# GBATZOLIS/ID-diff

Hardware: AMD Instinct MI355X
Metric: score-vector evals/sec (rows of S per second incl. the per-point spectrum), 32x32 ncsnpp (higher is better)
Workload: dtype f32 (3x3 convs: Winograd, fp32 transforms, contraction on pairs of fp16 values -- 22 significand bits, 3 products, fp32 accumulate (F(4,3) along the rows x 3 filter rows); 1x1/attention/dense contractions: fp32 operands split exactly into 3 bf16, 6 partial products, fp32 accumulate; the q/k/v projec

## Files before the change

id-diff_amd/_lib.py:

```python
import ctypes
import os
import subprocess

import torch

_HERE = os.path.dirname(os.path.abspath(__file__))
_VARIANT = os.environ.get("IDIFF_LIB_VARIANT", "")
_LIB_PATH = os.path.join(_HERE, "csrc", f"libidiff_hip.{_VARIANT}.so" if _VARIANT else "libidiff_hip.so")
_lib = None

ACT = {None: 0, "none": 0, "linear": 0, "silu": 1, "swish": 1, "elu": 2, "relu": 3, "lrelu": 4}

c_i, c_i64, c_f, c_p = ctypes.c_int, ctypes.c_int64, ctypes.c_float, ctypes.c_void_p


class Epilogue(ctypes.Structure):
    _fields_ = [("bias", c_p), ("rowbias", c_p), ("ld_rowbias", c_i64), ("rows_per_group", c_i), ("act", c_i),
                ("residual", c_p), ("ld_residual", c_i64), ("out_scale", c_f), ("rowscale", c_p), ("colstats", c_p)]


_SIGNATURES = {
    "idiff_abi_version": (c_i, []),
    "idiff_last_error": (ctypes.c_char_p, []),
    "idiff_source_stamp": (ctypes.c_char_p, []),
# ... 29 lines not shown
    "idiff_winograd43_pack_f32": (c_i, [c_p, c_p, c_i, c_i, c_p]),
    "idiff_conv2d_winograd43_f32": (c_i, [c_p, c_p, c_p, c_i, c_i, c_i, c_i, c_i, ctypes.POINTER(Epilogue), c_p]),
    "idiff_conv2d_winograd43h_ok": (c_i, [c_i] * 5),
    "idiff_winograd43h_weight_floats": (c_i64, [c_i, c_i]),
    "idiff_winograd43h_pack_f32": (c_i, [c_p, c_p, c_i, c_i, c_p]),
    "idiff_conv2d_winograd43h_f32": (c_i, [c_p, c_p, c_p, c_i, c_i, c_i, c_i, c_i, ctypes.POINTER(Epilogue), c_p]),
    "idiff_conv2d_wino1d_ok": (c_i, [c_i] * 5),
    "idiff_conv2d_wino1d_colstats_split": (c_i, [c_i] * 5),
    "idiff_wino1d_weight_floats": (c_i64, [c_i, c_i]),
    "idiff_wino1d_pack_f32": (c_i, [c_p, c_p, c_i, c_i, c_p]),
    "idiff_conv2d_wino1d_f32": (c_i, [c_p, c_p, c_p, c_i, c_i, c_i, c_i, c_i, ctypes.POINTER(Epilogue), c_p]),
    "idiff_conv2d_wino1d_gn_ok": (c_i, [c_i] * 6),
    "idiff_conv2d_wino1d_gn_f32": (c_i, [c_p, c_p, c_p, c_i, c_i, c_i, c_i, c_i, ctypes.POINTER(Epilogue), c_i, c_p, c_p, c_f, c_i, c_p]),
    "idiff_conv2d_winograd_split_ok": (c_i, [c_i] * 5),
    "idiff_winograd_split_weight_floats": (c_i64, [c_i, c_i]),
    "idiff_winograd_pack_split_f32": (c_i, [c_p, c_p, c_i, c_i, c_p]),
    "idiff_conv2d_winograd_split_f32": (c_i, [c_p, c_p, c_p] + [c_i] * 5 + [ctypes.POINTER(Epilogue), c_p]),
    "idiff_groupnorm_finalize_f32": (c_i, [c_p, c_i, c_i, c_p, c_i, c_i, c_i, c_i, c_i, c_f, c_p, c_p]),
    "idiff_groupnorm_nsplit": (c_i, [c_i, c_i, c_i]),
    "idiff_groupnorm_stats_f32": (c_i, [c_p, c_i, c_p, c_i, c_i, c_i, c_i, c_f, c_p, c_p, c_p]),
    "idiff_groupnorm_apply_f32": (c_i, [c_p, c_i, c_p, c_i, c_i, c_i, c_i, c_p, c_p, c_p, c_p, c_i64, c_i, c_p, c_p]),
    "idiff_groupnorm_apply_colstats_f32": (c_i, [c_p, c_i, c_p, c_i, c_i, c_i, c_i, c_p, c_i, c_p, c_i, c_f, c_p, c_p, c_p, c_i64,
                                                 c_i, c_p, c_p]),
    "idiff_softmax_rows_f32": (c_i, [c_p, c_p, c_i64, c_i, c_f, c_p]),
    "idiff_attention256_ok": (c_i, [c_i, c_i, c_i]),
    "idiff_attention256_f32": (c_i, [c_p, c_i64, c_p, c_p, c_p, c_p, c_p, c_i, c_i, c_i, c_f, c_p]),
    "idiff_attention_heads_ok": (c_i, [c_i, c_i, c_i, c_i]),
    "idiff_attention_heads_f32": (c_i, [c_p, c_i64, c_p, c_p, c_p, c_p, c_p, c_i, c_i, c_i, c_i, c_f, c_p]),
    "idiff_affine_act_f32": (c_i, [c_p, c_p, c_i64, c_f, c_f, c_i, c_p, c_i64, c_p]),
    "idiff_add_scale_f32": (c_i, [c_p, c_p, c_p, c_i64, c_f, c_p]),
    "idiff_fourier_embed_f32": (c_i, [c_p, c_p, c_p, c_i, c_i, c_p]),
    "idiff_positional_embed_f32": (c_i, [c_p, c_p, c_i, c_i, c_f, c_i, c_p]),
    "idiff_concat_cols_f32": (c_i, [c_p, c_i, c_p, c_i, c_p, c_i64, c_p]),
    "idiff_nchw_to_nhwc_f32": (c_i, [c_p, c_p, c_i, c_i, c_i, c_i, c_f, c_f, c_p]),
    "idiff_nhwc_to_nchw_f32": (c_i, [c_p, c_p, c_i, c_i, c_i, c_i, c_p, c_p]),
    "idiff_resample2x_nhwc_f32": (c_i, [c_p, c_p, c_i, c_i, c_i, c_i, c_i, c_p]),
    "idiff_perturb_f32": (c_i, [c_p, c_p, c_p, c_p, c_p, c_i64, c_i64, c_p]),
    "idiff_perturb_randn_f32": (c_i, [c_p, c_p, c_p, c_p, c_i64, c_i64, c_i64, ctypes.c_uint64, c_p, c_p]),
    "idiff_spectrum_workspace_bytes": (c_i64, [c_i, c_i, c_i]),
    "idiff_spectrum_f32": (c_i, [c_p, c_i, c_i, c_i, c_p, c_i64, c_p, c_p, c_p]),
    "idiff_colmean_f64": (c_i, [c_p, c_i, c_i, c_i, c_p, c_p, c_p]),
    "idiff_centered_gram_f64": (c_i, [c_p, c_p, c_i, c_i, c_i, c_p, c_p]),
    "idiff_centered_gram_rows_f64": (c_i, [c_p, c_p, c_i, c_i, c_i, c_i, c_p, c_p]),
    "idiff_symmetrize_upper_f64": (c_i, [c_p, c_i, c_p]),
    "idiff_symtridiag_scratch_doubles": (c_i64, [c_i]),
    "idiff_symband_ld": (c_i, []),
# ... 417 lines not shown
def groupnorm_nsplit(B, HW, C):
    return lib().idiff_groupnorm_nsplit(B, HW, C)


def groupnorm_stats(x, C, x2, C2, B, HW, G, eps, workspace, stats):
    _check(lib().idiff_groupnorm_stats_f32(x.data_ptr(), C, _ptr(x2), C2, B, HW, G, eps, workspace.data_ptr(),
                                           stats.data_ptr(), _stream()), "idiff_groupnorm_stats_f32")


def groupnorm_apply(x, C, x2, C2, B, HW, G, stats, gamma, beta, act, y, mod=None):
    _check(lib().idiff_groupnorm_apply_f32(x.data_ptr(), C, _ptr(x2), C2, B, HW, G, stats.data_ptr(), gamma.data_ptr(),
                                           beta.data_ptr(), _ptr(mod), mod.stride(0) if mod is not None else 0,
                                           ACT[act], y.data_ptr(), _stream()),
           "idiff_groupnorm_apply_f32")


def groupnorm_apply_colstats(x, C, x2, C2, B, HW, G, ws1, ns1, ws2, ns2, eps, gamma, beta, act, y, mod=None):
    _check(lib().idiff_groupnorm_apply_colstats_f32(x.data_ptr(), C, _ptr(x2), C2, B, HW, G, ws1.data_ptr(), ns1, _ptr(ws2), ns2,
                                                    eps, gamma.data_ptr(), beta.data_ptr(), _ptr(mod),
                                                    mod.stride(0) if mod is not None else 0, ACT[act], y.data_ptr(), _stream()),
           "idiff_groupnorm_apply_colstats_f32")


def softmax_rows(x, y, rows, cols, scale):
    _check(lib().idiff_softmax_rows_f32(x.data_ptr(), y.data_ptr(), rows, cols, scale, _stream()),
           "idiff_softmax_rows_f32")


def attention256_ok(B, tokens, C):
    return bool(lib().idiff_attention256_ok(B, tokens, C))


def pairs_scale_from_rows(w, bias=None, extra=1.0):
    ms = (w.double() ** 2).sum(dim=1).mean() * float(extra) ** 2
    if bias is not None:
        ms = ms + (bias.double() ** 2).mean()
    e = torch.round(-0.5 * torch.log2(ms.clamp_min(1e-300))).clamp(-24, 24)
    s = torch.exp2(e)
    return torch.stack([s, 1.0 / s]).to(torch.float32).contiguous()


def attention256(qk, vt, out, B, C, s_qk, s_v, scale, bias_v=None):
    _dev(qk, "qk"); _dev(vt, "vt"); _dev(out, "out"); _dev(s_qk, "s_qk"); _dev(s_v, "s_v")
    if qk.shape != (B * 256, 2 * C) or vt.shape != (B, C, 256) or out.numel() != B * 256 * C:
        raise RuntimeError(f"attention256: shapes qk {tuple(qk.shape)}, vt {tuple(vt.shape)}, out {tuple(out.shape)} for B = {B}, C = {C}")
    _check(lib().idiff_attention256_f32(qk.data_ptr(), qk.stride(0), vt.data_ptr(), _ptr(bias_v), s_qk.data_ptr(), s_v.data_ptr(),
# ... 264 lines not shown
```

id-diff_amd/csrc/common.h:

```cpp
#pragma once
#include <hip/hip_runtime.h>
#include <stdint.h>
#include <stdio.h>
#include <stdarg.h>

#include "../../include/idiff_hip.h"

#define IDIFF_API extern "C" __attribute__((visibility("default")))

namespace idiff {

void set_error(const char *fmt, ...);

inline int fail(const char *fmt, ...) {
  char buf[512];
  va_list ap;
  va_start(ap, fmt);
  vsnprintf(buf, sizeof(buf), fmt, ap);
  va_end(ap);
  set_error("%s", buf);
  return IDIFF_EINVAL;
}

inline int launch_status(const char *what) {
  hipError_t e = hipGetLastError();
  if (e != hipSuccess) {
    set_error("%s: %s", what, hipGetErrorString(e));
    return (int)e;
  }
  return 0;
}

enum Option { OPT_NO_WINOGRAD, OPT_NO_COLSTATS, OPT_NO_PIPE, OPT_SCALAR_EPILOGUE, OPT_DBUF_ONLY, OPT_TRIDIAG_ONESTAGE,
              OPT_UFD_ROWS, OPT_CHASE_WAVEFRONT, OPT_WINO_NGROUP, OPT_GRAM_SMALL_TILES, OPT_CHASE_SPIN_LIMIT, OPT_FAKE_CU_COUNT,
              OPT_SBR_SYNC, OPT_SBR_FULL, OPT_NO_SPLIT, OPT_WINO_SPLIT, OPT_SBR_LOOKAHEAD, OPT_NO_WINO43, OPT_NO_WINO43H, OPT_NO_PAIRS, OPT_PAIRS_MIN_TILES, OPT_NO_FUSED_ATTN, OPT_NO_WINO1D, OPT_NO_FUSED_GN, OPT_COUNT };
bool option(Option o);
int option_value(Option o);

struct AttrGuard { unsigned long long done_mask = 0; };
int set_dynamic_lds_once(AttrGuard &g, const void *const *fns, int n_fns, int bytes, const char *what);

bool conv3x3_narrow_ok(int B, int H, int W, int Cin, int Cout, int KH, int KW, int stride, int pad_lo, int pad_hi,
                       const idiff_epilogue *ep);
int conv3x3_narrow(const float *x, const float *wt, float *out, int B, int H, int W, int Cin, int Cout,
                   const idiff_epilogue *ep, hipStream_t stream);

template <class P> inline void set_epilogue(P &p, const idiff_epilogue *ep) {
  p.has_ep = ep ? 1 : 0;
  p.ep = ep ? *ep : idiff_epilogue{};
  if (!ep) p.ep.out_scale = 1.f;
  if (p.ep.rows_per_group <= 0) p.ep.rows_per_group = 1;
}

static inline int ceil_div(int a, int b) { return (a + b - 1) / b; }
static inline int64_t ceil_div64(int64_t a, int64_t b) { return (a + b - 1) / b; }

static inline int streaming_grid(int64_t work_items, int block) {
  int64_t g = ceil_div64(work_items, block);
// ... 18 lines not shown
```

id-diff_amd/csrc/norm_act.hip:

```cpp
#include "common.h"
#include <math.h>

namespace {

using idiff::act_apply;

__global__ void __launch_bounds__(256)
gn_partial_kernel(const float *__restrict__ x, int C, int c_off, int Ctot, int HW, int nsplit,
                  double *__restrict__ ws ) {
  __shared__ double red[256 * 8];
  const int b = blockIdx.x / nsplit, sp = blockIdx.x % nsplit;
  const int CV = C >> 2;
  const int RP = 256 / CV;
  const int tid = threadIdx.x;
  const int r0 = tid / CV, c4 = tid - r0 * CV;
  const int rows_per = (HW + nsplit - 1) / nsplit;
  const int row_lo = sp * rows_per, row_hi = min(HW, row_lo + rows_per);
  double s[4] = {0, 0, 0, 0}, q[4] = {0, 0, 0, 0};
  if (r0 < RP) {
    const float4 *xp = reinterpret_cast<const float4 *>(x) + (int64_t)b * HW * CV + c4;
    for (int r = row_lo + r0; r < row_hi; r += RP) {
      const float4 v = xp[(int64_t)r * CV];
      s[0] += v.x; q[0] += (double)v.x * v.x;
      s[1] += v.y; q[1] += (double)v.y * v.y;
      s[2] += v.z; q[2] += (double)v.z * v.z;
      s[3] += v.w; q[3] += (double)v.w * v.w;
    }
  }
// ... 59 lines not shown
    float4 in;
    if (c < C) in = *reinterpret_cast<const float4 *>(x + pix * C + c);
    else in = *reinterpret_cast<const float4 *>(x2 + pix * C2 + (c - C));
    const float4 ga = *reinterpret_cast<const float4 *>(gamma + c);
    const float4 be = *reinterpret_cast<const float4 *>(beta + c);
    float o[4] = {in.x, in.y, in.z, in.w};
    const float gg[4] = {ga.x, ga.y, ga.z, ga.w}, bb[4] = {be.x, be.y, be.z, be.w};
#pragma unroll
    for (int j = 0; j < 4; ++j) {
      const float *st = stats + 2 * ((int64_t)b * G + (c + j) / cpg);
      float v = (o[j] - st[0]) * st[1] * gg[j] + bb[j];
      if (mod) v = v * (1.0f + mod[(int64_t)b * ld_mod + c + j]) + mod[(int64_t)b * ld_mod + Ctot + c + j];
      o[j] = act_apply(v, act);
    }
    reinterpret_cast<float4 *>(y)[v] = make_float4(o[0], o[1], o[2], o[3]);
  }
}

__global__ void __launch_bounds__(256)
gn_apply_rows_kernel(const float *__restrict__ x, int C, const float *__restrict__ x2, int C2, int HW, int G,
                     const float *__restrict__ stats, const float *__restrict__ gamma, const float *__restrict__ beta,
                     const float *__restrict__ mod, int64_t ld_mod, int act, float *__restrict__ y, int rows_per_block,
                     const double *__restrict__ ws1, int ns1, const double *__restrict__ ws2, int ns2, float eps) {
  const int Ctot = C + C2, CVt = Ctot >> 2, cpg = Ctot / G;
  const int RP = 256 / CVt;
  const int tid = threadIdx.x;
  const int b = blockIdx.y;
  __shared__ float sh_stats[2 * 256];
  const bool shared_stats = ws1 != nullptr && G <= 256;
  if (shared_stats) {
    if (tid < G) {
      double sum = 0, sq = 0;
      for (int cc = tid * cpg; cc < (tid + 1) * cpg; ++cc) {
        const bool first = cc < C;
        const double *w = first ? ws1 + ((int64_t)b * ns1 * C + cc) * 2 : ws2 + ((int64_t)b * ns2 * C2 + (cc - C)) * 2;
        const int ns = first ? ns1 : ns2, Cs = first ? C : C2;
        for (int sp = 0; sp < ns; ++sp) { sum += w[(int64_t)sp * Cs * 2]; sq += w[(int64_t)sp * Cs * 2 + 1]; }
      }
      const double n = (double)cpg * HW;
      const double mean = sum / n;
      double var = sq / n - mean * mean;
      if (var < 0) var = 0;
      sh_stats[2 * tid] = (float)mean;
      sh_stats[2 * tid + 1] = (float)(1.0 / sqrt(var + (double)eps));
    }
    __syncthreads();
  }
  const int r0 = tid / CVt, c4 = tid - r0 * CVt;
  if (r0 >= RP) return;
  const int c = c4 * 4;
  float mu[4], s[4], t[4];
  float st_mean[4], st_rstd[4];
  if (shared_stats) {
#pragma unroll
    for (int j = 0; j < 4; ++j) { st_mean[j] = sh_stats[2 * ((c + j) / cpg)]; st_rstd[j] = sh_stats[2 * ((c + j) / cpg) + 1]; }
  } else if (ws1) {
    int g_prev = -1;
#pragma unroll
    for (int j = 0; j < 4; ++j) {
      const int g = (c + j) / cpg;
      if (g != g_prev) {
        double sum = 0, sq = 0;
        for (int cc = g * cpg; cc < (g + 1) * cpg; ++cc) {
          const bool first = cc < C;
          const double *w = first ? ws1 + ((int64_t)b * ns1 * C + cc) * 2 : ws2 + ((int64_t)b * ns2 * C2 + (cc - C)) * 2;
          const int ns = first ? ns1 : ns2, Cs = first ? C : C2;
          for (int sp = 0; sp < ns; ++sp) { sum += w[(int64_t)sp * Cs * 2]; sq += w[(int64_t)sp * Cs * 2 + 1]; }
        }
        const double n = (double)cpg * HW;
        const double mean = sum / n;
        double var = sq / n - mean * mean;
        if (var < 0) var = 0;
        st_mean[j] = (float)mean;
        st_rstd[j] = (float)(1.0 / sqrt(var + (double)eps));
        g_prev = g;
      } else {
        st_mean[j] = st_mean[j - 1]; st_rstd[j] = st_rstd[j - 1];
      }
    }
  } else {
#pragma unroll
    for (int j = 0; j < 4; ++j) {
      const float *st = stats + 2 * ((int64_t)b * G + (c + j) / cpg);
      st_mean[j] = st[0]; st_rstd[j] = st[1];
    }
  }
#pragma unroll
  for (int j = 0; j < 4; ++j) {
    const float st[2] = {st_mean[j], st_rstd[j]};
    float sc = st[1] * gamma[c + j], sh = beta[c + j];
    if (mod) {
      const float m1 = 1.0f + mod[(int64_t)b * ld_mod + c + j];
      sc *= m1;
      sh = sh * m1 + mod[(int64_t)b * ld_mod + Ctot + c + j];
    }
    mu[j] = st[0]; s[j] = sc; t[j] = sh;
  }
  const bool first = c < C;
  const float4 *src = first ? reinterpret_cast<const float4 *>(x + (int64_t)b * HW * C + c)
                            : reinterpret_cast<const float4 *>(x2 + (int64_t)b * HW * C2 + (c - C));
  const int src_stride = (first ? C : C2) >> 2;
  float4 *dst = reinterpret_cast<float4 *>(y + (int64_t)b * HW * Ctot + c);
  const int p_lo = blockIdx.x * rows_per_block, p_hi = min(HW, p_lo + rows_per_block);
  int p = p_lo + r0;
  for (; p + 3 * RP < p_hi; p += 4 * RP) {
    float4 v[4];
#pragma unroll
    for (int u = 0; u < 4; ++u) {
      v[u] = src[(int64_t)(p + u * RP) * src_stride];
    }
#pragma unroll
    for (int u = 0; u < 4; ++u) {
      float4 o;
      o.x = act_apply((v[u].x - mu[0]) * s[0] + t[0], act);
      o.y = act_apply((v[u].y - mu[1]) * s[1] + t[1], act);
      o.z = act_apply((v[u].z - mu[2]) * s[2] + t[2], act);
      o.w = act_apply((v[u].w - mu[3]) * s[3] + t[3], act);
      dst[(int64_t)(p + u * RP) * CVt] = o;
    }
  }
  for (; p < p_hi; p += RP) {
    const float4 v = src[(int64_t)p * src_stride];
    float4 o;
    o.x = act_apply((v.x - mu[0]) * s[0] + t[0], act);
    o.y = act_apply((v.y - mu[1]) * s[1] + t[1], act);
    o.z = act_apply((v.z - mu[2]) * s[2] + t[2], act);
    o.w = act_apply((v.w - mu[3]) * s[3] + t[3], act);
    dst[(int64_t)p * CVt] = o;
  }
}

__device__ __forceinline__ float wave_max(float v) {
#pragma unroll
  for (int o = 32; o > 0; o >>= 1) v = fmaxf(v, __shfl_xor(v, o, 64));
  return v;
}
__device__ __forceinline__ float wave_sum(float v) {
#pragma unroll
  for (int o = 32; o > 0; o >>= 1) v += __shfl_xor(v, o, 64);
  return v;
}

__global__ void __launch_bounds__(256)
softmax_rows_kernel(const float *__restrict__ x, float *__restrict__ y, int64_t rows, int cols, float scale) {
  const int lane = threadIdx.x & 63;
  const int64_t row = (int64_t)blockIdx.x * 4 + (threadIdx.x >> 6);
  if (row >= rows) return;
  const float *xr = x + row * cols;
  float *yr = y + row * cols;
  constexpr int PL = 16;
  if (cols <= 64 * PL) {
// ... 442 lines not shown
```

id-diff_amd/csrc/runtime.hip:

```cpp
#include "common.h"
#include <stdlib.h>
#include <string.h>
#include <limits.h>

namespace idiff {
static thread_local char g_err[512] = "";
void set_error(const char *fmt, ...) {
  va_list ap;
  va_start(ap, fmt);
  vsnprintf(g_err, sizeof(g_err), fmt, ap);
  va_end(ap);
}

namespace {
const char *const kOptionNames[OPT_COUNT] = {"IDIFF_NO_WINOGRAD", "IDIFF_NO_COLSTATS", "IDIFF_NO_PIPE", "IDIFF_SCALAR_EPILOGUE",
                                             "IDIFF_DBUF_ONLY", "IDIFF_TRIDIAG_ONESTAGE", "IDIFF_UFD_ROWS", "IDIFF_CHASE_WAVEFRONT",
                                             "IDIFF_WINO_NGROUP", "IDIFF_GRAM_SMALL_TILES", "IDIFF_CHASE_SPIN_LIMIT",
                                             "IDIFF_FAKE_CU_COUNT", "IDIFF_SBR_SYNC", "IDIFF_SBR_FULL", "IDIFF_NO_SPLIT", "IDIFF_WINO_SPLIT", "IDIFF_SBR_LOOKAHEAD",
                                             "IDIFF_NO_WINO43", "IDIFF_NO_WINO43H", "IDIFF_NO_PAIRS", "IDIFF_PAIRS_MIN_TILES", "IDIFF_NO_FUSED_ATTN", "IDIFF_NO_WINO1D", "IDIFF_NO_FUSED_GN"};
struct OptionTable {
  int v[OPT_COUNT];
  OptionTable() {
    for (int i = 0; i < OPT_COUNT; ++i) { const char *e = getenv(kOptionNames[i]); v[i] = (e && *e) ? atoi(e) : 0; }
  }
};
OptionTable g_options;
constexpr int kUnset = INT_MIN;
struct ThreadOptions {
  int v[OPT_COUNT];
  ThreadOptions() { for (int i = 0; i < OPT_COUNT; ++i) v[i] = kUnset; }
};
thread_local ThreadOptions t_options;
}

int option_value(Option o) {
  const int t = t_options.v[o];
  return t != kUnset ? t : __atomic_load_n(&g_options.v[o], __ATOMIC_RELAXED);
}
bool option(Option o) { return option_value(o) != 0; }

int set_dynamic_lds_once(AttrGuard &g, const void *const *fns, int n_fns, int bytes, const char *what) {
  int dev = 0;
// ... 40 lines not shown
```

id-diff_amd/csrc/upfirdn2d.hip:

```cpp
#include "common.h"
#include <stdlib.h>
#include <algorithm>

namespace {

struct UfdParams {
  int major, in_h, in_w, minor, kh, kw;
  int up_x, up_y, down_x, down_y, pad_x0, pad_y0;
  int out_h, out_w;
};

__device__ __forceinline__ int floor_div(int a, int b) {
  int q = a / b;
  return (a % b != 0 && a < 0) ? q - 1 : q;
}
__device__ __forceinline__ int ceil_div_s(int a, int b) { return -floor_div(-a, b); }

constexpr int kMaxTaps = 64;

struct GroupPlan { int ppb, grid, ngroups; };
template <typename LdsBytes, typename Admissible>
GroupPlan plan_plane_groups(int major, int ppb_max, LdsBytes lds_bytes_of, Admissible admissible) {
  if (lds_bytes_of(1) > 64 * 1024) return {0, 0, 0};
  GroupPlan best = {1, major, major};
// ... 449 lines not shown
#pragma unroll
      for (int c = 0; c < 3; ++c) {
        const int ix = j - 1 + c;
        const bool ok = vy && (unsigned)ix < (unsigned)p.in_w;
        in[r][c] = ok ? xp[((int64_t)iy * p.in_w + ix) * cv] : zero;
      }
    }
#pragma unroll
    for (int a = 0; a < 2; ++a)
#pragma unroll
      for (int b = 0; b < 2; ++b) {
        float4 acc = zero;
#pragma unroll
        for (int u = 0; u < 2; ++u)
#pragma unroll
          for (int v = 0; v < 2; ++v) {
            const float wt = w[(a + 2 * u) * 4 + (b + 2 * v)];
            const float4 sv = in[a + u][b + v];
            acc.x += sv.x * wt; acc.y += sv.y * wt; acc.z += sv.z * wt; acc.w += sv.w * wt;
          }
        op[((int64_t)a * p.out_w + 2 * j + b) * cv] = acc;
      }
  }
}

__global__ void __launch_bounds__(256)
upfirdn2d_generic(const float *__restrict__ x, const float *__restrict__ k, float *__restrict__ out, UfdParams p,
                  int64_t total) {
  for (int64_t v = (int64_t)blockIdx.x * blockDim.x + threadIdx.x; v < total; v += (int64_t)gridDim.x * blockDim.x) {
    int c = (int)(v % p.minor);
    int64_t pix = v / p.minor;
    int ox = (int)(pix % p.out_w);
    int64_t t = pix / p.out_w;
    int oy = (int)(t % p.out_h);
    int64_t plane = t / p.out_h;
    const int by = oy * p.down_y - p.pad_y0, bx = ox * p.down_x - p.pad_x0;
    const int iy_lo = max(ceil_div_s(by, p.up_y), 0), iy_hi = min(floor_div(by + p.kh - 1, p.up_y), p.in_h - 1);
    const int ix_lo = max(ceil_div_s(bx, p.up_x), 0), ix_hi = min(floor_div(bx + p.kw - 1, p.up_x), p.in_w - 1);
    float acc = 0.f;
    for (int iy = iy_lo; iy <= iy_hi; ++iy) {
      const int ky = iy * p.up_y - by;
      for (int ix = ix_lo; ix <= ix_hi; ++ix) {
        const int kx = ix * p.up_x - bx;
        acc += x[((plane * p.in_h + iy) * p.in_w + ix) * p.minor + c] * k[(p.kh - 1 - ky) * p.kw + (p.kw - 1 - kx)];
      }
    }
// ... 239 lines not shown
      hipLaunchKernelGGL(upfirdn2d_nhwc_rows<1>, c.grid, blk, 0, st, x, k, out, p, c.cv, c.col_step);
      return launch_status("upfirdn2d_nhwc_rows");
    case UFD_NHWC_ROWS_ANY:
      hipLaunchKernelGGL(upfirdn2d_nhwc_rows<-1>, c.grid, blk, 0, st, x, k, out, p, c.cv, c.col_step);
      return launch_status("upfirdn2d_nhwc_rows");
    case UFD_NHWC_VEC4:
      hipLaunchKernelGGL(upfirdn2d_nhwc_vec4, c.grid, blk, 0, st, x, k, out, p, c.total);
      return launch_status("upfirdn2d_nhwc_vec4");
    case UFD_GENERIC:
      hipLaunchKernelGGL(upfirdn2d_generic, c.grid, blk, 0, st, x, k, out, p, c.total);
      return launch_status("upfirdn2d_generic");
  }
  return fail("upfirdn2d: no route");
}

IDIFF_API const char *idiff_upfirdn2d_route(const void *x, const void *out, int major, int in_h, int in_w, int minor, int kh, int kw,
                                            int up_x, int up_y, int down_x, int down_y, int pad_x0, int pad_x1, int pad_y0,
                                            int pad_y1) {
  UfdParams p;
  UfdPlan c;
  if (ufd_choose(x, out, major, in_h, in_w, minor, kh, kw, up_x, up_y, down_x, down_y, pad_x0, pad_x1, pad_y0, pad_y1, p, c)) return nullptr;
  return kUfdRouteNames[c.route];
}
```

id-diff_amd/models/ncsnpp.py:

```python
import math

import numpy as np
import torch
import torch.nn as nn

from .. import _lib
from . import utils
from .nhwc import NhwcExecutor, _T, _pad4

_INV_SQRT2 = float(1.0 / np.sqrt(2.0))


def _fan_avg_uniform(shape, scale=1.):
    scale = 1e-10 if scale == 0 else scale
    rf = np.prod(shape) / shape[1] / shape[0]
    variance = scale / ((shape[1] * rf + shape[0] * rf) / 2)
    return (torch.rand(*shape) * 2. - 1.) * np.sqrt(3 * variance)


def _conv(cin, cout, k, init_scale=1., stride=1, padding=None):
    conv = nn.Conv2d(cin, cout, k, stride=stride, padding=(k // 2 if padding is None else padding))
    conv.weight.data = _fan_avg_uniform(conv.weight.shape, init_scale)
    nn.init.zeros_(conv.bias)
    return conv
# ... 247 lines not shown
            pk["nin"][key] = (self._pack_nin(nin, cin_split), nin.b.detach().float().contiguous())
        return pk["nin"][key]

    def _fir(self, x, pk, mode):
        B = x.buf.shape[0]
        n = pk["fir_len"]
        if mode == "up":
            p = n - 2
            k, up, down, p0, p1 = pk["fir_up"], 2, 1, (p + 1) // 2 + 1, p // 2
        elif mode == "down":
            p = n - 2
            k, up, down, p0, p1 = pk["fir_down"], 1, 2, (p + 1) // 2, p // 2
        else:
            p = (n - 2) + 2
            k, up, down, p0, p1 = pk["fir_down"], 1, 1, (p + 1) // 2, p // 2
        OH = _lib.upfirdn2d_out_size(x.H, up, down, p0, p1, n)
        OW = _lib.upfirdn2d_out_size(x.W, up, down, p0, p1, n)
        y = self._new(B, OH, OW, x.C, x.buf)
        _lib.upfirdn2d_raw(x.buf, k, y.buf, B, x.H, x.W, x.C, up, up, down, down, p0, p1, p0, p1)
        if x.norm is not None:
            y.norm = (x.norm[0], x.norm[1], x.norm[2] * pk["fir_gain"][mode], x.norm[3])
        return y

    def _resblock(self, idx, x, temb_all, pk, x2=None):
        mod = self.all_modules[idx]
        rs = _INV_SQRT2 if self.skip_rescale else 1.0
        c_in = x.C + (x2.C if x2 is not None else 0)
        assert c_in == mod.in_ch, (c_in, mod.in_ch)
        h = self._gn_act(x, mod.GroupNorm_0, self.act_name, x2)
        if mod.up or mod.down:
            assert x2 is None
            if self.fir:
                h, x = self._fir(h, pk, "up" if mod.up else "down"), self._fir(x, pk, "up" if mod.up else "down")
            else:
                h, x = self._box(h, mod.up), self._box(x, mod.up)
        w0, b0 = self._conv_w(pk, (idx, 0), mod.Conv_0)
        off = pk["dense_off"][idx]
        h = self._conv_gn_act(h, w0, b0, mod.GroupNorm_1, self.act_name, rowbias=temb_all[:, off:off + mod.out_ch], normed=True)
        if hasattr(mod, "Conv_2") or hasattr(mod, "NIN_0"):
            fused = x2 is not None and x.C == x2.C and x.C % 32 == 0
            split = x.C if (x2 is not None and not fused) else None
            if hasattr(mod, "Conv_2"):
                ws, bs = self._conv_w(pk, (idx, 2), mod.Conv_2, split)
                ws = [w.view(w.shape[0], -1) for w in ws] if split is not None else ws.view(ws.shape[0], -1)
            else:
                ws, bs = self._nin_w(pk, (idx, "nin"), mod.NIN_0, split)
            if x2 is None:
                sc = self._pointwise(x, ws, bs)
            elif fused:
                sc = self._new(x.buf.shape[0], x.H, x.W, ws.shape[0], x.buf)
                _lib.gemm_2src(x.buf.view(-1, x.C), x2.buf.view(-1, x2.C), ws, sc.buf.view(-1, ws.shape[0]),
                               epilogue=_lib.make_epilogue(bias=bs))
            else:
                part = self._pointwise(x, ws[0], bs)
                sc = self._pointwise(x2, ws[1], None, residual=part.buf)
        else:
            assert x2 is None
            sc = x
# ... 132 lines not shown
```

include/idiff_hip.h:

```cpp
#ifndef IDIFF_HIP_H
#define IDIFF_HIP_H

#include <stdint.h>

#ifdef __cplusplus
extern "C" {
#endif

#define IDIFF_EINVAL 1001
#define IDIFF_ABI_VERSION 1

int idiff_abi_version(void);
const char *idiff_last_error(void);
const char *idiff_source_stamp(void);
const char *idiff_variant_flags(void);

int idiff_set_option(const char *name, int value);

int idiff_set_thread_option(const char *name, int value, int set);


int idiff_upfirdn2d_f32(const float *x, const float *k, float *out, int major, int in_h, int in_w, int minor,
                        int kh, int kw, int up_x, int up_y, int down_x, int down_y, int pad_x0, int pad_x1,
                        int pad_y0, int pad_y1, void *stream);
// ... 87 lines not shown
                               const idiff_epilogue *ep, int groups, const float *gamma, const float *beta, float eps, int act,
                               void *stream);

int idiff_conv2d_winograd_split_ok(int B, int H, int W, int Cin, int Cout);
int64_t idiff_winograd_split_weight_floats(int Cin, int Cout);
int idiff_winograd_pack_split_f32(const float *wt, float *u, int Cin, int Cout, void *stream);
int idiff_conv2d_winograd_split_f32(const float *x, const float *u, float *out, int B, int H, int W, int Cin, int Cout,
                                    const idiff_epilogue *ep, void *stream);


int idiff_groupnorm_nsplit(int B, int HW, int C);
int idiff_groupnorm_stats_f32(const float *x, int C, const float *x2, int C2, int B, int HW, int G, float eps,
                              double *workspace, float *stats, void *stream);
int idiff_groupnorm_finalize_f32(const double *ws1, int nsplit1, int C1, const double *ws2, int nsplit2, int C2, int B,
                                 int HW, int G, float eps, float *stats, void *stream);
int idiff_groupnorm_apply_f32(const float *x, int C, const float *x2, int C2, int B, int HW, int G,
                              const float *stats, const float *gamma, const float *beta, const float *mod,
                              int64_t ld_mod, int act, float *y, void *stream);
int idiff_groupnorm_apply_colstats_f32(const float *x, int C, const float *x2, int C2, int B, int HW, int G,
                                       const double *ws1, int nsplit1, const double *ws2, int nsplit2, float eps,
                                       const float *gamma, const float *beta, const float *mod, int64_t ld_mod,
                                       int act, float *y, void *stream);

int idiff_softmax_rows_f32(const float *x, float *y, int64_t rows, int cols, float scale, void *stream);

int idiff_attention256_ok(int B, int tokens, int C);
int idiff_attention256_f32(const float *qk, int64_t ld_qk, const float *vt, const float *bias_v, const float *s_qk, const float *s_v,
                           float *out, int B, int tokens, int C, float scale, void *stream);

int idiff_attention_heads_ok(int B, int tokens, int H, int D);
int idiff_attention_heads_f32(const float *qk, int64_t ld_qk, const float *vt, const float *bias_v, const float *s_qk, const float *s_v,
                              float *out, int B, int tokens, int H, int D, float scale, void *stream);

int idiff_affine_act_f32(const float *a, float *y, int64_t n, float alpha, float beta_const, int act,
                         const float *rowscale, int64_t inner, void *stream);
int idiff_add_scale_f32(const float *a, const float *b, float *y, int64_t n, float scale, void *stream);
int idiff_fourier_embed_f32(const float *t, const float *W, float *out, int B, int half, void *stream);
int idiff_positional_embed_f32(const float *t, float *out, int B, int dim, float max_positions, int mode, void *stream);
int idiff_concat_cols_f32(const float *a, int Ca, const float *b, int Cb, float *out, int64_t rows, void *stream);
int idiff_nchw_to_nhwc_f32(const float *x, float *y, int B, int C, int HW, int Cpad, float alpha, float beta,
                           void *stream);
int idiff_nhwc_to_nchw_f32(const float *x, float *y, int B, int C, int HW, int Cpad, const float *rowscale,
                           void *stream);
int idiff_perturb_f32(const float *x, const float *z, const float *std_, const float *mean_coeff, float *out,
                      int64_t rows, int64_t D, void *stream);
int idiff_perturb_randn_f32(const float *x, const float *std_, const float *mean_coeff, float *out, int64_t rows,
// ... 33 lines not shown
```

Measured before the change: 17820.

## Fuse GroupNorm+activation with both FIR resamples in up/down resblocks

Adds a kernel that applies GroupNorm and the activation and runs the 4x4 FIR up- or down-sampling on both the normalized branch and the skip input in one pass. Resblocks that resample now call it instead of separate norm-apply and two FIR launches. The goal is to avoid writing and re-reading the full-resolution normalized map and to cut launches. The shared GN helpers are factored into a header, and an env option can switch the fused path off.

```diff
diff --git a/id-diff_amd/_lib.py b/id-diff_amd/_lib.py
--- a/id-diff_amd/_lib.py
+++ b/id-diff_amd/_lib.py
@@ -75,6 +75,8 @@
     "idiff_groupnorm_apply_f32": (c_i, [c_p, c_i, c_p, c_i, c_i, c_i, c_i, c_p, c_p, c_p, c_p, c_i64, c_i, c_p, c_p]),
     "idiff_groupnorm_apply_colstats_f32": (c_i, [c_p, c_i, c_p, c_i, c_i, c_i, c_i, c_p, c_i, c_p, c_i, c_f, c_p, c_p, c_p, c_i64,
                                                  c_i, c_p, c_p]),
+    "idiff_gn_act_fir2_ok": (c_i, [c_i] * 6),
+    "idiff_gn_act_fir2_f32": (c_i, [c_p, c_p, c_p] + [c_i] * 7 + [c_p, c_p, c_i, c_f, c_p, c_p, c_p, c_i, c_i, c_p, c_p, c_p]),
     "idiff_softmax_rows_f32": (c_i, [c_p, c_p, c_i64, c_i, c_f, c_p]),
     "idiff_attention256_ok": (c_i, [c_i, c_i, c_i]),
     "idiff_attention256_f32": (c_i, [c_p, c_i64, c_p, c_p, c_p, c_p, c_p, c_i, c_i, c_i, c_f, c_p]),
@@ -538,6 +540,25 @@
            "idiff_groupnorm_apply_colstats_f32")
 
 
+FIR2_MODE = {"down": 0, "up": 1}
+
+
+def gn_act_fir2_ok(B, H, W, C, G, mode, taps=4, x2=None, mod=None):
+    if taps != 4 or x2 is not None or mod is not None or mode not in FIR2_MODE:
+        return False
+    return bool(lib().idiff_gn_act_fir2_ok(B, H, W, C, G, FIR2_MODE[mode]))
+
+
+def gn_act_fir2(x, k, B, H, W, C, G, eps, gamma, beta, act, mode, hr, xr, stats=None, colstats=None, x2=None, mod=None):
+    ws1, ns1 = colstats if colstats is not None else (None, 0)
+    if mode not in FIR2_MODE:
+        raise ValueError(f"gn_act_fir2: mode {mode!r} (down or up)")
+    kh, kw = k.shape
+    _check(lib().idiff_gn_act_fir2_f32(x.data_ptr(), _ptr(x2), k.data_ptr(), kh, kw, B, H, W, C, G, _ptr(stats), _ptr(ws1), ns1, eps,
+                                       gamma.data_ptr(), beta.data_ptr(), _ptr(mod), ACT[act], FIR2_MODE[mode], hr.data_ptr(),
+                                       xr.data_ptr(), _stream()), "idiff_gn_act_fir2_f32")
+
+
 def softmax_rows(x, y, rows, cols, scale):
     _check(lib().idiff_softmax_rows_f32(x.data_ptr(), y.data_ptr(), rows, cols, scale, _stream()),
            "idiff_softmax_rows_f32")
diff --git a/id-diff_amd/csrc/common.h b/id-diff_amd/csrc/common.h
--- a/id-diff_amd/csrc/common.h
+++ b/id-diff_amd/csrc/common.h
@@ -33,7 +33,7 @@
 
 enum Option { OPT_NO_WINOGRAD, OPT_NO_COLSTATS, OPT_NO_PIPE, OPT_SCALAR_EPILOGUE, OPT_DBUF_ONLY, OPT_TRIDIAG_ONESTAGE,
               OPT_UFD_ROWS, OPT_CHASE_WAVEFRONT, OPT_WINO_NGROUP, OPT_GRAM_SMALL_TILES, OPT_CHASE_SPIN_LIMIT, OPT_FAKE_CU_COUNT,
-              OPT_SBR_SYNC, OPT_SBR_FULL, OPT_NO_SPLIT, OPT_WINO_SPLIT, OPT_SBR_LOOKAHEAD, OPT_NO_WINO43, OPT_NO_WINO43H, OPT_NO_PAIRS, OPT_PAIRS_MIN_TILES, OPT_NO_FUSED_ATTN, OPT_NO_WINO1D, OPT_NO_FUSED_GN, OPT_COUNT };
+              OPT_SBR_SYNC, OPT_SBR_FULL, OPT_NO_SPLIT, OPT_WINO_SPLIT, OPT_SBR_LOOKAHEAD, OPT_NO_WINO43, OPT_NO_WINO43H, OPT_NO_PAIRS, OPT_PAIRS_MIN_TILES, OPT_NO_FUSED_ATTN, OPT_NO_WINO1D, OPT_NO_FUSED_GN, OPT_NO_GN_FIR, OPT_COUNT };
 bool option(Option o);
 int option_value(Option o);
 
diff --git a/id-diff_amd/csrc/gn_common.h b/id-diff_amd/csrc/gn_common.h
--- /dev/null
+++ b/id-diff_amd/csrc/gn_common.h
@@ -0,0 +1,86 @@
+#pragma once
+#include "common.h"
+#include <math.h>
+
+namespace idiff {
+
+__device__ __forceinline__ void gn_group_from_colsums(const double *__restrict__ ws1, int ns1, int C, const double *__restrict__ ws2,
+                                                      int ns2, int C2, int b, int g, int cpg, int HW, float eps, float &mean_out,
+                                                      float &rstd_out) {
+  double sum = 0, sq = 0;
+  for (int cc = g * cpg; cc < (g + 1) * cpg; ++cc) {
+    const bool first = cc < C;
+    const double *w = first ? ws1 + ((int64_t)b * ns1 * C + cc) * 2 : ws2 + ((int64_t)b * ns2 * C2 + (cc - C)) * 2;
+    const int ns = first ? ns1 : ns2, Cs = first ? C : C2;
+    for (int sp = 0; sp < ns; ++sp) { sum += w[(int64_t)sp * Cs * 2]; sq += w[(int64_t)sp * Cs * 2 + 1]; }
+  }
+  const double n = (double)cpg * HW;
+  const double mean = sum / n;
+  double var = sq / n - mean * mean;
+  if (var < 0) var = 0;
+  mean_out = (float)mean;
+  rstd_out = (float)(1.0 / sqrt(var + (double)eps));
+}
+
+__device__ __forceinline__ bool gn_stats_to_lds(float *sh_stats, int tid, int b, int C, int C2, int G, int HW,
+                                                const double *__restrict__ ws1, int ns1, const double *__restrict__ ws2, int ns2,
+                                                float eps) {
+  const bool shared_stats = ws1 != nullptr && G <= 256;
+  if (shared_stats) {
+    if (tid < G) gn_group_from_colsums(ws1, ns1, C, ws2, ns2, C2, b, tid, (C + C2) / G, HW, eps, sh_stats[2 * tid], sh_stats[2 * tid + 1]);
+    __syncthreads();
+  }
+  return shared_stats;
+}
+
+__device__ __forceinline__ void gn_column_constants(const float *sh_stats, bool shared_stats, int b, int c, int C, int C2, int G, int HW,
+                                                    const float *__restrict__ stats, const float *__restrict__ gamma,
+                                                    const float *__restrict__ beta, const float *__restrict__ mod, int64_t ld_mod,
+                                                    const double *__restrict__ ws1, int ns1, const double *__restrict__ ws2, int ns2,
+                                                    float eps, float (&mu)[4], float (&s)[4], float (&t)[4]) {
+  const int Ctot = C + C2, cpg = Ctot / G;
+  float st_mean[4], st_rstd[4];
+  if (shared_stats) {
+#pragma unroll
+    for (int j = 0; j < 4; ++j) { st_mean[j] = sh_stats[2 * ((c + j) / cpg)]; st_rstd[j] = sh_stats[2 * ((c + j) / cpg) + 1]; }
+  } else if (ws1) {
+    int g_prev = -1;
+#pragma unroll
+    for (int j = 0; j < 4; ++j) {
+      const int g = (c + j) / cpg;
+      if (g != g_prev) {
+        gn_group_from_colsums(ws1, ns1, C, ws2, ns2, C2, b, g, cpg, HW, eps, st_mean[j], st_rstd[j]);
+        g_prev = g;
+      } else {
+        st_mean[j] = st_mean[j - 1]; st_rstd[j] = st_rstd[j - 1];
+      }
+    }
+  } else {
+#pragma unroll
+    for (int j = 0; j < 4; ++j) {
+      const float *st = stats + 2 * ((int64_t)b * G + (c + j) / cpg);
+      st_mean[j] = st[0]; st_rstd[j] = st[1];
+    }
+  }
+#pragma unroll
+  for (int j = 0; j < 4; ++j) {
+    float sc = st_rstd[j] * gamma[c + j], sh = beta[c + j];
+    if (mod) {
+      const float m1 = 1.0f + mod[(int64_t)b * ld_mod + c + j];
+      sc *= m1;
+      sh = sh * m1 + mod[(int64_t)b * ld_mod + Ctot + c + j];
+    }
+    mu[j] = st_mean[j]; s[j] = sc; t[j] = sh;
+  }
+}
+
+__device__ __forceinline__ float4 gn_column_apply(const float4 v, const float (&mu)[4], const float (&s)[4], const float (&t)[4], int act) {
+  float4 o;
+  o.x = act_apply((v.x - mu[0]) * s[0] + t[0], act);
+  o.y = act_apply((v.y - mu[1]) * s[1] + t[1], act);
+  o.z = act_apply((v.z - mu[2]) * s[2] + t[2], act);
+  o.w = act_apply((v.w - mu[3]) * s[3] + t[3], act);
+  return o;
+}
+
+}
diff --git a/id-diff_amd/csrc/norm_act.hip b/id-diff_amd/csrc/norm_act.hip
--- a/id-diff_amd/csrc/norm_act.hip
+++ b/id-diff_amd/csrc/norm_act.hip
@@ -1,9 +1,13 @@
 #include "common.h"
+#include "gn_common.h"
 #include <math.h>
 
 namespace {
 
 using idiff::act_apply;
+using idiff::gn_stats_to_lds;
+using idiff::gn_column_constants;
+using idiff::gn_column_apply;
 
 __global__ void __launch_bounds__(256)
 gn_partial_kernel(const float *__restrict__ x, int C, int c_off, int Ctot, int HW, int nsplit,
@@ -109,80 +113,17 @@
                      const float *__restrict__ stats, const float *__restrict__ gamma, const float *__restrict__ beta,
                      const float *__restrict__ mod, int64_t ld_mod, int act, float *__restrict__ y, int rows_per_block,
                      const double *__restrict__ ws1, int ns1, const double *__restrict__ ws2, int ns2, float eps) {
-  const int Ctot = C + C2, CVt = Ctot >> 2, cpg = Ctot / G;
+  const int Ctot = C + C2, CVt = Ctot >> 2;
   const int RP = 256 / CVt;
   const int tid = threadIdx.x;
   const int b = blockIdx.y;
   __shared__ float sh_stats[2 * 256];
-  const bool shared_stats = ws1 != nullptr && G <= 256;
-  if (shared_stats) {
-    if (tid < G) {
-      double sum = 0, sq = 0;
-      for (int cc = tid * cpg; cc < (tid + 1) * cpg; ++cc) {
-        const bool first = cc < C;
-        const double *w = first ? ws1 + ((int64_t)b * ns1 * C + cc) * 2 : ws2 + ((int64_t)b * ns2 * C2 + (cc - C)) * 2;
-        const int ns = first ? ns1 : ns2, Cs = first ? C : C2;
-        for (int sp = 0; sp < ns; ++sp) { sum += w[(int64_t)sp * Cs * 2]; sq += w[(int64_t)sp * Cs * 2 + 1]; }
-      }
-      const double n = (double)cpg * HW;
-      const double mean = sum / n;
-      double var = sq / n - mean * mean;
-      if (var < 0) var = 0;
-      sh_stats[2 * tid] = (float)mean;
-      sh_stats[2 * tid + 1] = (float)(1.0 / sqrt(var + (double)eps));
-    }
-    __syncthreads();
-  }
+  const bool shared_stats = gn_stats_to_lds(sh_stats, tid, b, C, C2, G, HW, ws1, ns1, ws2, ns2, eps);
   const int r0 = tid / CVt, c4 = tid - r0 * CVt;
   if (r0 >= RP) return;
   const int c = c4 * 4;
   float mu[4], s[4], t[4];
-  float st_mean[4], st_rstd[4];
-  if (shared_stats) {
-#pragma unroll
-    for (int j = 0; j < 4; ++j) { st_mean[j] = sh_stats[2 * ((c + j) / cpg)]; st_rstd[j] = sh_stats[2 * ((c + j) / cpg) + 1]; }
-  } else if (ws1) {
-    int g_prev = -1;
-#pragma unroll
-    for (int j = 0; j < 4; ++j) {
-      const int g = (c + j) / cpg;
-      if (g != g_prev) {
-        double sum = 0, sq = 0;
-        for (int cc = g * cpg; cc < (g + 1) * cpg; ++cc) {
-          const bool first = cc < C;
-          const double *w = first ? ws1 + ((int64_t)b * ns1 * C + cc) * 2 : ws2 + ((int64_t)b * ns2 * C2 + (cc - C)) * 2;
-          const int ns = first ? ns1 : ns2, Cs = first ? C : C2;
-          for (int sp = 0; sp < ns; ++sp) { sum += w[(int64_t)sp * Cs * 2]; sq += w[(int64_t)sp * Cs * 2 + 1]; }
-        }
-        const double n = (double)cpg * HW;
-        const double mean = sum / n;
-        double var = sq / n - mean * mean;
-        if (var < 0) var = 0;
-        st_mean[j] = (float)mean;
-        st_rstd[j] = (float)(1.0 / sqrt(var + (double)eps));
-        g_prev = g;
-      } else {
-        st_mean[j] = st_mean[j - 1]; st_rstd[j] = st_rstd[j - 1];
-      }
-    }
-  } else {
-#pragma unroll
-    for (int j = 0; j < 4; ++j) {
-      const float *st = stats + 2 * ((int64_t)b * G + (c + j) / cpg);
-      st_mean[j] = st[0]; st_rstd[j] = st[1];
-    }
-  }
-#pragma unroll
-  for (int j = 0; j < 4; ++j) {
-    const float st[2] = {st_mean[j], st_rstd[j]};
-    float sc = st[1] * gamma[c + j], sh = beta[c + j];
-    if (mod) {
-      const float m1 = 1.0f + mod[(int64_t)b * ld_mod + c + j];
-      sc *= m1;
-      sh = sh * m1 + mod[(int64_t)b * ld_mod + Ctot + c + j];
-    }
-    mu[j] = st[0]; s[j] = sc; t[j] = sh;
-  }
+  gn_column_constants(sh_stats, shared_stats, b, c, C, C2, G, HW, stats, gamma, beta, mod, ld_mod, ws1, ns1, ws2, ns2, eps, mu, s, t);
   const bool first = c < C;
   const float4 *src = first ? reinterpret_cast<const float4 *>(x + (int64_t)b * HW * C + c)
                             : reinterpret_cast<const float4 *>(x2 + (int64_t)b * HW * C2 + (c - C));
@@ -198,22 +139,12 @@
     }
 #pragma unroll
     for (int u = 0; u < 4; ++u) {
-      float4 o;
-      o.x = act_apply((v[u].x - mu[0]) * s[0] + t[0], act);
-      o.y = act_apply((v[u].y - mu[1]) * s[1] + t[1], act);
-      o.z = act_apply((v[u].z - mu[2]) * s[2] + t[2], act);
-      o.w = act_apply((v[u].w - mu[3]) * s[3] + t[3], act);
-      dst[(int64_t)(p + u * RP) * CVt] = o;
+      dst[(int64_t)(p + u * RP) * CVt] = gn_column_apply(v[u], mu, s, t, act);
     }
   }
   for (; p < p_hi; p += RP) {
     const float4 v = src[(int64_t)p * src_stride];
-    float4 o;
-    o.x = act_apply((v.x - mu[0]) * s[0] + t[0], act);
-    o.y = act_apply((v.y - mu[1]) * s[1] + t[1], act);
-    o.z = act_apply((v.z - mu[2]) * s[2] + t[2], act);
-    o.w = act_apply((v.w - mu[3]) * s[3] + t[3], act);
-    dst[(int64_t)p * CVt] = o;
+    dst[(int64_t)p * CVt] = gn_column_apply(v, mu, s, t, act);
   }
 }
 
diff --git a/id-diff_amd/csrc/runtime.hip b/id-diff_amd/csrc/runtime.hip
--- a/id-diff_amd/csrc/runtime.hip
+++ b/id-diff_amd/csrc/runtime.hip
@@ -17,7 +17,7 @@
                                              "IDIFF_DBUF_ONLY", "IDIFF_TRIDIAG_ONESTAGE", "IDIFF_UFD_ROWS", "IDIFF_CHASE_WAVEFRONT",
                                              "IDIFF_WINO_NGROUP", "IDIFF_GRAM_SMALL_TILES", "IDIFF_CHASE_SPIN_LIMIT",
                                              "IDIFF_FAKE_CU_COUNT", "IDIFF_SBR_SYNC", "IDIFF_SBR_FULL", "IDIFF_NO_SPLIT", "IDIFF_WINO_SPLIT", "IDIFF_SBR_LOOKAHEAD",
-                                             "IDIFF_NO_WINO43", "IDIFF_NO_WINO43H", "IDIFF_NO_PAIRS", "IDIFF_PAIRS_MIN_TILES", "IDIFF_NO_FUSED_ATTN", "IDIFF_NO_WINO1D", "IDIFF_NO_FUSED_GN"};
+                                             "IDIFF_NO_WINO43", "IDIFF_NO_WINO43H", "IDIFF_NO_PAIRS", "IDIFF_PAIRS_MIN_TILES", "IDIFF_NO_FUSED_ATTN", "IDIFF_NO_WINO1D", "IDIFF_NO_FUSED_GN", "IDIFF_NO_GN_FIR"};
 struct OptionTable {
   int v[OPT_COUNT];
   OptionTable() {
diff --git a/id-diff_amd/csrc/upfirdn2d.hip b/id-diff_amd/csrc/upfirdn2d.hip
--- a/id-diff_amd/csrc/upfirdn2d.hip
+++ b/id-diff_amd/csrc/upfirdn2d.hip
@@ -1,4 +1,5 @@
 #include "common.h"
+#include "gn_common.h"
 #include <stdlib.h>
 #include <algorithm>
 
@@ -495,6 +496,170 @@
         op[((int64_t)a * p.out_w + 2 * j + b) * cv] = acc;
       }
   }
+}
+
+struct GnFirParams {
+  const float *x, *k, *stats, *gamma, *beta;
+  const double *ws1;
+  float *hr, *xr;
+  int ns1, act, H, W, C, G, cv, OH, OW;
+  int rows, blocks_per_plane;
+  float eps;
+};
+
+#define GN_FIR_PROLOGUE                                                                                                           \
+  __shared__ float sh_stats[2 * 256];                                                                                             \
+  __shared__ float taps[16];                                                                                                      \
+  const int tid = threadIdx.x, cv = p.cv, W = p.W;                                                                                \
+  if (tid < 16) taps[tid] = p.k[(3 - (tid >> 2)) * 4 + (3 - (tid & 3))];                                                          \
+  const int bid = xcd_contiguous(blockIdx.x, gridDim.x);                                                                          \
+  const int b = bid / p.blocks_per_plane, rb = bid - b * p.blocks_per_plane;                                                      \
+  const bool shared_stats = idiff::gn_stats_to_lds(sh_stats, tid, b, p.C, 0, p.G, p.H * W, p.ws1, p.ns1, p.ws1, 0, p.eps);        \
+  __syncthreads();                                                                                                                \
+  const int r0 = tid / cv, c4 = tid - r0 * cv;                                                                                    \
+  if (r0 >= 256 / cv) return;                                                                                                     \
+  float mu[4], s[4], t[4];                                                                                                        \
+  idiff::gn_column_constants(sh_stats, shared_stats, b, 4 * c4, p.C, 0, p.G, p.H * W, p.stats, p.gamma, p.beta, nullptr, 0, p.ws1, \
+                             p.ns1, p.ws1, 0, p.eps, mu, s, t);                                                                   \
+  float w[16];                                                \
+  _Pragma("unroll") for (int i = 0; i < 16; ++i)                                                                                  \
+    w[i] = __builtin_bit_cast(float, __builtin_amdgcn_readfirstlane(__builtin_bit_cast(int, taps[i])));                           \
+  const float4 zero = make_float4(0.f, 0.f, 0.f, 0.f);                                                                            \
+  const float4 *xp = reinterpret_cast<const float4 *>(p.x) + (int64_t)b * p.H * W * cv + c4
+
+__global__ void __launch_bounds__(256)
+gn_act_fir_down2_kernel(GnFirParams p) {
+  GN_FIR_PROLOGUE;
+  const int oy = rb * p.rows + r0;
+  if (oy >= p.OH) return;
+  const int64_t o0 = ((int64_t)b * p.OH + oy) * p.OW * cv + c4;
+  float4 *ho = reinterpret_cast<float4 *>(p.hr) + o0, *xo = reinterpret_cast<float4 *>(p.xr) + o0;
+  bool vy[4];
+  const float4 *row[4];
+  float4 xs[4][4], hs[4][4];
+#pragma unroll
+  for (int ky = 0; ky < 4; ++ky) {
+    const int iy = 2 * oy - 1 + ky;
+    vy[ky] = (unsigned)iy < (unsigned)p.H;
+    row[ky] = xp + (int64_t)(vy[ky] ? iy : 0) * W * cv;
+    const float4 v = row[ky][0];
+    xs[ky][2] = zero; hs[ky][2] = zero;
+    xs[ky][3] = vy[ky] ? v : zero;
+    hs[ky][3] = vy[ky] ? idiff::gn_column_apply(v, mu, s, t, p.act) : zero;
+  }
+#pragma unroll 2
+  for (int ox = 0; ox < p.OW; ++ox) {
+    const int ix2 = 2 * ox + 1, ix3 = 2 * ox + 2;
+    const bool v2 = ix2 < W, v3 = ix3 < W;
+    const int64_t a2 = (int64_t)min(ix2, W - 1) * cv, a3 = (int64_t)min(ix3, W - 1) * cv;
+    float4 n2[4], n3[4];
+#pragma unroll
+    for (int ky = 0; ky < 4; ++ky) { n2[ky] = row[ky][a2]; n3[ky] = row[ky][a3]; }
+#pragma unroll
+    for (int ky = 0; ky < 4; ++ky) {
+      xs[ky][0] = xs[ky][2]; xs[ky][1] = xs[ky][3]; hs[ky][0] = hs[ky][2]; hs[ky][1] = hs[ky][3];
+      const bool ok2 = vy[ky] && v2, ok3 = vy[ky] && v3;
+      xs[ky][2] = ok2 ? n2[ky] : zero;
+      xs[ky][3] = ok3 ? n3[ky] : zero;
+      hs[ky][2] = ok2 ? idiff::gn_column_apply(n2[ky], mu, s, t, p.act) : zero;
+      hs[ky][3] = ok3 ? idiff::gn_column_apply(n3[ky], mu, s, t, p.act) : zero;
+    }
+    float4 ax = zero, ah = zero;
+#pragma unroll
+    for (int ky = 0; ky < 4; ++ky)
+#pragma unroll
+      for (int kx = 0; kx < 4; ++kx) {
+        const float wt = w[ky * 4 + kx];
+        const float4 sv = xs[ky][kx], hv = hs[ky][kx];
+        ax.x += sv.x * wt; ax.y += sv.y * wt; ax.z += sv.z * wt; ax.w += sv.w * wt;
+        ah.x += hv.x * wt; ah.y += hv.y * wt; ah.z += hv.z * wt; ah.w += hv.w * wt;
+      }
+    xo[(int64_t)ox * cv] = ax;
+    ho[(int64_t)ox * cv] = ah;
+  }
+}
+
+__device__ __forceinline__ void gn_fir_load_row(float4 (&xrow)[3], float4 (&hrow)[3], const float4 *xp, int iy, int iy_valid, int H,
+                                                int row_pitch, const int64_t (&ax)[3], const bool (&vx)[3], const float (&mu)[4],
+                                                const float (&s)[4], const float (&t)[4], int act) {
+  const bool vy = (unsigned)iy < (unsigned)H;
+  const float4 *row = xp + (int64_t)(vy ? iy : iy_valid) * row_pitch;
+#pragma unroll
+  for (int c = 0; c < 3; ++c) {
+    const float4 v = row[ax[c]];
+    const bool ok = vy && vx[c];
+    xrow[c] = ok ? v : make_float4(0.f, 0.f, 0.f, 0.f);
+    hrow[c] = ok ? idiff::gn_column_apply(v, mu, s, t, act) : make_float4(0.f, 0.f, 0.f, 0.f);
+  }
+}
+
+__global__ void __launch_bounds__(256)
+gn_act_fir_up2_kernel(GnFirParams p) {
+  GN_FIR_PROLOGUE;
+  const int col_step = 256 / cv, i0 = rb * p.rows, i1 = min(p.H, i0 + p.rows);
+  for (int j = r0; j < W; j += col_step) {
+    bool vx[3];
+    int64_t ax[3];
+#pragma unroll
+    for (int c = 0; c < 3; ++c) {
+      const int ix = j - 1 + c;
+      vx[c] = (unsigned)ix < (unsigned)W;
+      ax[c] = (int64_t)(vx[c] ? ix : j) * cv;
+    }
+    float4 xs[3][3], hs[3][3];
+    gn_fir_load_row(xs[1], hs[1], xp, i0 - 1, i0, p.H, W * cv, ax, vx, mu, s, t, p.act);
+    gn_fir_load_row(xs[2], hs[2], xp, i0, i0, p.H, W * cv, ax, vx, mu, s, t, p.act);
+#pragma unroll 2
+    for (int i = i0; i < i1; ++i) {
+#pragma unroll
+      for (int c = 0; c < 3; ++c) { xs[0][c] = xs[1][c]; xs[1][c] = xs[2][c]; hs[0][c] = hs[1][c]; hs[1][c] = hs[2][c]; }
+      gn_fir_load_row(xs[2], hs[2], xp, i + 1, i0, p.H, W * cv, ax, vx, mu, s, t, p.act);
+      const int64_t o0 = (((int64_t)b * p.OH + 2 * i) * p.OW + 2 * j) * cv + c4;
+      float4 *ho = reinterpret_cast<float4 *>(p.hr) + o0, *xo = reinterpret_cast<float4 *>(p.xr) + o0;
+#pragma unroll
+      for (int a = 0; a < 2; ++a)
+#pragma unroll
+        for (int bb = 0; bb < 2; ++bb) {
+          float4 accx = zero, acch = zero;
+#pragma unroll
+          for (int u = 0; u < 2; ++u)
+#pragma unroll
+            for (int v = 0; v < 2; ++v) {
+              const float wt = w[(a + 2 * u) * 4 + (bb + 2 * v)];
+              const float4 sv = xs[a + u][bb + v], hv = hs[a + u][bb + v];
+              accx.x += sv.x * wt; accx.y += sv.y * wt; accx.z += sv.z * wt; accx.w += sv.w * wt;
+              acch.x += hv.x * wt; acch.y += hv.y * wt; acch.z += hv.z * wt; acch.w += hv.w * wt;
+            }
+          xo[((int64_t)a * p.OW + bb) * cv] = accx;
+          ho[((int64_t)a * p.OW + bb) * cv] = acch;
+        }
+    }
+  }
+}
+#undef GN_FIR_PROLOGUE
+
+const char *gn_fir_plan(int B, int H, int W, int C, int G, int mode, GnFirParams &p, unsigned &grid) {
+  if (B <= 0 || H <= 0 || W <= 0 || C <= 0 || G <= 0) return "bad shape";
+  if (mode != IDIFF_FIR2_DOWN && mode != IDIFF_FIR2_UP) return "mode must be IDIFF_FIR2_DOWN or IDIFF_FIR2_UP";
+  if (C % 4 != 0 || C > 1024) return "channels must be a multiple of 4 and at most 1024";
+  if (C % G != 0 || G > 256) return "groups must divide the channels and be at most 256";
+  if (mode == IDIFF_FIR2_DOWN && (H < 2 || W < 2)) return "a map of fewer than 2 x 2 pixels has no decimated output";
+  if ((int64_t)H * W > (1 << 24)) return "map too large";
+  p.H = H; p.W = W; p.C = C; p.G = G; p.cv = C / 4;
+  if (mode == IDIFF_FIR2_DOWN) {
+    p.OH = (H - 2) / 2 + 1; p.OW = (W - 2) / 2 + 1;
+    p.rows = 256 / p.cv;
+  } else {
+    p.OH = 2 * H; p.OW = 2 * W;
+    p.rows = 1;
+    for (int r = 4; r > 1; r >>= 1)
+      if (r <= H && (int64_t)B * idiff::ceil_div(H, r) >= 2048) { p.rows = r; break; }
+  }
+  p.blocks_per_plane = idiff::ceil_div(mode == IDIFF_FIR2_DOWN ? p.OH : H, p.rows);
+  const int64_t blocks = (int64_t)B * p.blocks_per_plane;
+  if (blocks > 0xffffffll) return "too many workgroups for one launch";
+  grid = (unsigned)blocks;
+  return nullptr;
 }
 
 __global__ void __launch_bounds__(256)
@@ -780,3 +945,32 @@
   if (ufd_choose(x, out, major, in_h, in_w, minor, kh, kw, up_x, up_y, down_x, down_y, pad_x0, pad_x1, pad_y0, pad_y1, p, c)) return nullptr;
   return kUfdRouteNames[c.route];
 }
+
+IDIFF_API int idiff_gn_act_fir2_ok(int B, int H, int W, int C, int G, int mode) {
+  if (idiff::option(idiff::OPT_NO_GN_FIR)) return 0;
+  GnFirParams p;
+  unsigned grid;
+  return gn_fir_plan(B, H, W, C, G, mode, p, grid) == nullptr;
+}
+
+IDIFF_API int idiff_gn_act_fir2_f32(const float *x, const float *x2, const float *k, int kh, int kw, int B, int H, int W, int C, int G,
+                                    const float *stats, const double *ws1, int nsplit1, float eps, const float *gamma,
+                                    const float *beta, const float *mod, int act, int mode, float *hr, float *xr, void *stream) {
+  using namespace idiff;
+  if (!x || !k || !gamma || !beta || !hr || !xr) return fail("gn_act_fir2: null pointer");
+  if (x2) return fail("gn_act_fir2: a second source is not served (GroupNorm apply and the two FIR launches are)");
+  if (mod) return fail("gn_act_fir2: a modulated norm is not served");
+  if (kh != 4 || kw != 4) return fail("gn_act_fir2: %d x %d taps (4 x 4 only)", kh, kw);
+  if ((stats != nullptr) == (ws1 != nullptr)) return fail("gn_act_fir2: the statistics come as stats or as column sums, one of the two");
+  if (ws1 && nsplit1 <= 0) return fail("gn_act_fir2: column sums need nsplit1 > 0");
+  if (option(OPT_NO_GN_FIR)) return fail("gn_act_fir2: switched off (IDIFF_NO_GN_FIR)");
+  GnFirParams p;
+  unsigned grid;
+  if (const char *why = gn_fir_plan(B, H, W, C, G, mode, p, grid)) return fail("gn_act_fir2: %s (B=%d %dx%d C=%d G=%d)", why, B, H, W, C, G);
+  if ((((uintptr_t)x | (uintptr_t)hr | (uintptr_t)xr) & 15) != 0) return fail("gn_act_fir2: x, hr and xr must be 16-byte aligned");
+  p.x = x; p.k = k; p.stats = stats; p.gamma = gamma; p.beta = beta; p.ws1 = ws1; p.ns1 = nsplit1; p.hr = hr; p.xr = xr;
+  p.act = act; p.eps = eps;
+  if (mode == IDIFF_FIR2_DOWN) hipLaunchKernelGGL(gn_act_fir_down2_kernel, dim3(grid), dim3(256), 0, (hipStream_t)stream, p);
+  else hipLaunchKernelGGL(gn_act_fir_up2_kernel, dim3(grid), dim3(256), 0, (hipStream_t)stream, p);
+  return launch_status(mode == IDIFF_FIR2_DOWN ? "gn_act_fir_down2" : "gn_act_fir_up2");
+}
diff --git a/id-diff_amd/models/ncsnpp.py b/id-diff_amd/models/ncsnpp.py
--- a/id-diff_amd/models/ncsnpp.py
+++ b/id-diff_amd/models/ncsnpp.py
@@ -293,18 +293,45 @@
             y.norm = (x.norm[0], x.norm[1], x.norm[2] * pk["fir_gain"][mode], x.norm[3])
         return y
 
+    def _gn_act_fir2(self, x, gn, act, pk, mode):
+        B = x.buf.shape[0]
+        G = gn.num_groups
+        k = pk["fir_up"] if mode == "up" else pk["fir_down"]
+        OH, OW = (2 * x.H, 2 * x.W) if mode == "up" else ((x.H - 2) // 2 + 1, (x.W - 2) // 2 + 1)
+        stats = colstats = None
+        if x.stats is not None:
+            colstats = x.stats
+        else:
+            nsplit = _lib.groupnorm_nsplit(B, x.H * x.W, x.C)
+            ws = torch.empty(B * nsplit * x.C * 2, device=x.buf.device, dtype=torch.float64)
+            stats = torch.empty(B * G * 2, device=x.buf.device, dtype=torch.float32)
+            _lib.groupnorm_stats(x.buf, x.C, None, 0, B, x.H * x.W, G, gn.eps, ws, stats)
+        h, xr = self._new(B, OH, OW, x.C, x.buf), self._new(B, OH, OW, x.C, x.buf)
+        _lib.gn_act_fir2(x.buf, k, B, x.H, x.W, x.C, G, gn.eps, gn.weight.detach(), gn.bias.detach(), act, mode, h.buf, xr.buf,
+                         stats=stats, colstats=colstats)
+        h.norm = (gn, (x.C // G) * x.H * x.W, 1.0 * pk["fir_gain"][mode], False)
+        if x.norm is not None:
+            xr.norm = (x.norm[0], x.norm[1], x.norm[2] * pk["fir_gain"][mode], x.norm[3])
+        return h, xr
+
     def _resblock(self, idx, x, temb_all, pk, x2=None):
         mod = self.all_modules[idx]
         rs = _INV_SQRT2 if self.skip_rescale else 1.0
         c_in = x.C + (x2.C if x2 is not None else 0)
         assert c_in == mod.in_ch, (c_in, mod.in_ch)
-        h = self._gn_act(x, mod.GroupNorm_0, self.act_name, x2)
         if mod.up or mod.down:
             assert x2 is None
-            if self.fir:
-                h, x = self._fir(h, pk, "up" if mod.up else "down"), self._fir(x, pk, "up" if mod.up else "down")
+            mode = "up" if mod.up else "down"
+            if self.fir and _lib.gn_act_fir2_ok(x.buf.shape[0], x.H, x.W, x.C, mod.GroupNorm_0.num_groups, mode, taps=pk["fir_len"]):
+                h, x = self._gn_act_fir2(x, mod.GroupNorm_0, self.act_name, pk, mode)
             else:
-                h, x = self._box(h, mod.up), self._box(x, mod.up)
+                h = self._gn_act(x, mod.GroupNorm_0, self.act_name)
+                if self.fir:
+                    h, x = self._fir(h, pk, mode), self._fir(x, pk, mode)
+                else:
+                    h, x = self._box(h, mod.up), self._box(x, mod.up)
+        else:
+            h = self._gn_act(x, mod.GroupNorm_0, self.act_name, x2)
         w0, b0 = self._conv_w(pk, (idx, 0), mod.Conv_0)
         off = pk["dense_off"][idx]
         h = self._conv_gn_act(h, w0, b0, mod.GroupNorm_1, self.act_name, rowbias=temb_all[:, off:off + mod.out_ch], normed=True)
diff --git a/include/idiff_hip.h b/include/idiff_hip.h
--- a/include/idiff_hip.h
+++ b/include/idiff_hip.h
@@ -133,6 +133,13 @@
                                        const float *gamma, const float *beta, const float *mod, int64_t ld_mod,
                                        int act, float *y, void *stream);
 
+#define IDIFF_FIR2_DOWN 0
+#define IDIFF_FIR2_UP 1
+int idiff_gn_act_fir2_ok(int B, int H, int W, int C, int G, int mode);
+int idiff_gn_act_fir2_f32(const float *x, const float *x2, const float *k, int kh, int kw, int B, int H, int W, int C, int G,
+                          const float *stats, const double *ws1, int nsplit1, float eps, const float *gamma, const float *beta,
+                          const float *mod, int act, int mode, float *hr, float *xr, void *stream);
+
 int idiff_softmax_rows_f32(const float *x, float *y, int64_t rows, int cols, float scale, void *stream);
 
 int idiff_attention256_ok(int B, int tokens, int C);
```

Result: no change. 17990, median of 6 (+0.9%).
